# MariusFurter/WeightedSampling.jl

Measured on NVIDIA B200. Metric: particle_updates_per_sec, higher is better.
Workload: dtype f64

## Files before the change

include/wsb200.h:

```cpp
#ifndef WSB200_H
#define WSB200_H

#include <stdint.h>

#ifdef __cplusplus
extern "C" {
#endif

#define WSB200_ABI_VERSION 2

#define WS_OK 0
#define WS_EINVAL (-1)
#define WS_ENODEVICE (-2)
#define WS_ECUDA (-3)
#define WS_ENOMEM (-4)
#define WS_EUNSUPPORTED (-5)
#define WS_EREPLAY (-6)
#define WS_ENUMERIC (-7)
#define WS_ENCCL (-8)

typedef struct ws_ctx ws_ctx;

#define WS_RESAMPLER_STRATIFIED 0
#define WS_RESAMPLER_SYSTEMATIC 1
// ... 194 lines not shown
    int64_t h2d_bytes;
    int64_t d2h_bytes;
    double last_resample_ms;
    double last_pass_ms;
    int64_t sl_passes;
} ws_stats;
int ws_get_stats(ws_ctx* ctx, ws_stats* out);
int ws_get_clamped(ws_ctx* ctx, int64_t* out);
int ws_get_ess_ties(ws_ctx* ctx, int64_t* out);
#define WS_N_KERNEL_CLASSES 8
int ws_kernel_times(ws_ctx* ctx, double* ms_out, int64_t* count_out, int32_t n_classes);
int ws_reset_kernel_times(ws_ctx* ctx);
int ws_set_lazy_gather(ws_ctx* ctx, int on);
typedef struct ws_plane_stats {
    double mean, median, std, min, max;
    double hist[8];
} ws_plane_stats;
int ws_describe(ws_ctx* ctx, int32_t n_planes, const int32_t* col, const int32_t* comp, ws_plane_stats* out, double* ess);

int ws_set_genealogy(ws_ctx* ctx, int on, int64_t budget_bytes);
int ws_genealogy_info(ws_ctx* ctx, int64_t* n_vectors, int64_t* bytes, int64_t* events);
int ws_col_events_behind(ws_ctx* ctx, int32_t id, int64_t* out);
int ws_set_timing(ws_ctx* ctx, int on);
int ws_get_migrated(ws_ctx* ctx, int64_t* out);
int ws_get_pushed(ws_ctx* ctx, int64_t* out);
int ws_get_mailbox_exchanges(ws_ctx* ctx, int64_t* out);
int ws_get_traced_pushes(ws_ctx* ctx, int64_t* out);
int ws_next_philox_stream(ws_ctx* ctx, uint64_t* stream_out, uint64_t* seed_out);
int ws_stream(ws_ctx* ctx, void** stream_out);

#ifdef __cplusplus
}
#endif
#endif
```

weightedsampling.jl_b200/_lib.py:

```python
from __future__ import annotations

import ctypes as C
import os

_HERE = os.path.dirname(os.path.abspath(__file__))
LIB_PATH = os.environ.get("WSB200_LIB", os.path.join(_HERE, "lib", "libwsb200.so"))


class WsError(RuntimeError):

    def __init__(self, code, msg):
        super().__init__(f"wsb200 error {code}: {msg}")
        self.code = code
        self.msg = msg


class UnsupportedModelError(WsError):
    """The statement is outside the fixed device-op set (rejected, never run on the CPU)."""


WS_OK, WS_EINVAL, WS_ENODEVICE, WS_ECUDA, WS_ENOMEM, WS_EUNSUPPORTED, WS_EREPLAY, WS_ENUMERIC, WS_ENCCL = (
    0, -1, -2, -3, -4, -5, -6, -7, -8)

RESAMPLER = {"stratified": 0, "systematic": 1, "multinomial": 2}
# ... 121 lines not shown
    "ws_marginal_diversity": (C.c_int, [_ctx, C.c_int32, _i32p, _i32p, _dp]),
    "ws_score_logpdf": (C.c_int, [_ctx, C.c_int64, C.c_void_p]),
    "ws_tape_clear": (C.c_int, [_ctx]),
    "ws_tape_record_only": (C.c_int, [_ctx, C.c_int]),
    "ws_tape_length": (C.c_int, [_ctx, _i64p]),
    "ws_tape_enable": (C.c_int, [_ctx, C.c_int]),
    "ws_set_replay_normals": (C.c_int, [_ctx, C.c_void_p, C.c_int64]),
    "ws_set_replay_uniforms": (C.c_int, [_ctx, C.c_void_p, C.c_int64]),
    "ws_set_replay_exponentials": (C.c_int, [_ctx, C.c_void_p, C.c_int64]),
    "ws_set_replay_variates": (C.c_int, [_ctx, C.c_void_p, C.c_int64]),
    "ws_get_stats": (C.c_int, [_ctx, C.POINTER(ws_stats)]),
    "ws_get_clamped": (C.c_int, [_ctx, _i64p]),
    "ws_get_ess_ties": (C.c_int, [_ctx, _i64p]),
    "ws_kernel_times": (C.c_int, [_ctx, _dp, _i64p, C.c_int32]),
    "ws_reset_kernel_times": (C.c_int, [_ctx]),
    "ws_set_timing": (C.c_int, [_ctx, C.c_int]),
    "ws_set_lazy_gather": (C.c_int, [_ctx, C.c_int]),
    "ws_describe": (C.c_int, [_ctx, C.c_int32, C.POINTER(C.c_int32), C.POINTER(C.c_int32), C.POINTER(ws_plane_stats),
                              C.POINTER(C.c_double)]),
    "ws_set_genealogy": (C.c_int, [_ctx, C.c_int, C.c_int64]),
    "ws_genealogy_info": (C.c_int, [_ctx, _i64p, _i64p, _i64p]),
    "ws_col_events_behind": (C.c_int, [_ctx, C.c_int32, _i64p]),
    "ws_next_philox_stream": (C.c_int, [_ctx, C.POINTER(C.c_uint64), C.POINTER(C.c_uint64)]),
    "ws_get_migrated": (C.c_int, [_ctx, _i64p]),
    "ws_get_pushed": (C.c_int, [_ctx, _i64p]),
    "ws_get_mailbox_exchanges": (C.c_int, [_ctx, _i64p]),
    "ws_get_traced_pushes": (C.c_int, [_ctx, _i64p]),
    "ws_stream": (C.c_int, [_ctx, C.POINTER(C.c_void_p)]),
}

_lib = None


def load():
    global _lib
    if _lib is not None:
        return _lib
    if not os.path.exists(LIB_PATH):
        raise ImportError(
            f"{LIB_PATH} is missing: build it with `python -c 'import __graft_entry__ as g; g.build()'` "
            "(nvcc, sm_100a).  wsb200 has no CPU fallback.")
    if "WSB200_NCCL_LIB" not in os.environ:
        import importlib.util
        spec = importlib.util.find_spec("nvidia")
        for base in (list(spec.submodule_search_locations) if spec and spec.submodule_search_locations else []):
            cand = os.path.join(base, "nccl", "lib", "libnccl.so.2")
# ... 23 lines not shown
```

weightedsampling.jl_b200/csrc/ws_kernels.cu:

```cuda
#include "ws_internal.h"

static int g_sm_count = 148;

__device__ __forceinline__ void lse_push(WsLse& a, double l) {
    if (l == -INFINITY) return;
    if (l > a.m) {
        double sc = ws_exp_nonpos(a.m - l);
        a.S = a.S * sc + 1.0;
        a.Q = a.Q * sc * sc + 1.0;
        a.m = l;
    } else {
        double e = ws_exp_nonpos(l - a.m);
        a.S += e;
        a.Q += e * e;
    }
}

template <int K>
__device__ __forceinline__ void lse_push_many(WsLse& a, const double (&l)[K], const bool (&live)[K]) {
    double mx = -INFINITY;
#pragma unroll
    for (int j = 0; j < K; ++j)
        if (live[j]) mx = fmax(mx, l[j]);
    if (mx > a.m) {
// ... 556 lines not shown
int ws_vm_max_grid(int n_regs, int n_loads, int n_ops, int sm_count, int n_ckpt) {
    const int smem = ws_vm_smem_bytes(n_regs, n_loads, n_ops, n_ckpt) + 1024;
    int per_sm = (227 * 1024) / smem;
    if (per_sm > WS_VM_MINB) per_sm = WS_VM_MINB;
    if (per_sm < 1) per_sm = 1;
    return per_sm * sm_count;
}

cudaError_t ws_launch_vm(const WsVmProgram& P, int grid, cudaStream_t s) {
    if (!g_vm_interp_only && P.n_ckpt == 0) {
        switch (ws_sl_find(P)) {
#define WS_SL_CASE(idx, Sig) \
    case idx: return ws_launch_vm_sl<Sig>(P, s);
            WS_SL_SIGS(WS_SL_CASE)
#undef WS_SL_CASE
            default: break;
        }
    }
    if (!g_vm_interp_only && P.n_ckpt != 0 && ws_slck_ok(P)) {
        constexpr int smem_ck = WsSigLinregObs::n_loads * WS_VM_BLOCK * WS_SLCK_P * (int)sizeof(double);
        ws_vm_sl_ckpt_kernel<WsSigLinregObs, WS_SLCK_P, WS_SLCK_N><<<ws_slck_grid(P), WS_VM_BLOCK, smem_ck, s>>>(P);
        return cudaGetLastError();
    }
    const int smem = ws_vm_smem_bytes(P.n_regs, P.n_loads, P.n_ops, P.n_ckpt);
    if (P.n_ckpt > 0) {
        if (ws_vm_staged(P.n_regs, P.n_loads)) ws_vm_kernel<true, true><<<grid, WS_VM_BLOCK, smem, s>>>(P);
        else ws_vm_kernel<false, true><<<grid, WS_VM_BLOCK, smem, s>>>(P);
    } else if (ws_vm_staged(P.n_regs, P.n_loads)) ws_vm_kernel<true><<<grid, WS_VM_BLOCK, smem, s>>>(P);
    else ws_vm_kernel<false><<<grid, WS_VM_BLOCK, smem, s>>>(P);
    return cudaGetLastError();
}

__global__ void __launch_bounds__(256) ws_reduce_logw_kernel(const double* __restrict__ logw, int64_t n,
                                                             WsLse* __restrict__ partials) {
    __shared__ WsLse warp_scratch[8];
    WsLse part;
    part.m = -INFINITY;
    part.S = 0.0;
    part.Q = 0.0;
    const int64_t stride = (int64_t)gridDim.x * 256;
    for (int64_t i = (int64_t)blockIdx.x * 256 + threadIdx.x; i < n; i += stride) lse_push(part, __ldg(logw + i));
    WsLse tot = lse_block_reduce<256>(part, warp_scratch);
    if (threadIdx.x == 0) partials[blockIdx.x] = tot;
}

cudaError_t ws_launch_reduce_logw(const double* logw, int64_t n, WsLse* partials, int grid, cudaStream_t s) {
    ws_reduce_logw_kernel<<<grid, 256, 0, s>>>(logw, n, partials);
    return cudaGetLastError();
}

__device__ __forceinline__ void ws_count_ess_tie(double ess, double ess_min, unsigned long long* ties) {
    if (ties != nullptr && fabs(ess - ess_min) <= 8.0 * 2.220446049250313e-16 * fabs(ess_min)) atomicAdd(ties, 1ull);
// ... 1967 lines not shown
```

weightedsampling.jl_b200/csrc/ws_lowering.h:

```cpp
#pragma once
#include <math.h>
#include <stdint.h>
#include <string.h>
#include <map>
#include <string>
#include <utility>
#include <vector>
#include "../../include/wsb200.h"
#include "ws_vm.cuh"

namespace wsl {

struct Plane {
    int32_t col, comp;
    bool operator<(const Plane& o) const { return col < o.col || (col == o.col && comp < o.comp); }
    bool operator==(const Plane& o) const { return col == o.col && comp == o.comp; }
};

struct Val {
    bool is_const;
    double c0, c1;
    int reg;
    static Val constant(double v) { return Val{true, v, 0.0, -1}; }
    static Val lin(double c0, double c1, int reg) { return Val{false, c0, c1, reg}; }
// ... 799 lines not shown
    const double K = (-0.5 * WS_LOG2PI - log(ts)) - (-0.5 * WS_LOG2PI - log(ps));
    p.has_acc = true;
    p.emit(ws_make_op(WS_OP_ACC_LIN2, 0, st.reg, sp.reg, WS_REG_NONE, 0, K, -0.5, 0.5));
}

inline void stmt_sample_expr(Program& p, RngCursor& rc, Plane dst, const ws_expr& sampler, const ws_expr* weighter) {
    p.rng = &rc;
    Val x = p.compile(sampler);
    p.rng = nullptr;
    p.store_val(dst, x);
    if (weighter != nullptr) p.acc_val(p.compile(*weighter));
}

inline bool mvnormal_factors(int d, const double* cov, std::vector<double>& L, std::vector<double>& Linv, double& c0) {
    if (!cholesky_lower(d, cov, L)) return false;
    lower_inverse(d, L, Linv);
    double logdet = 0.0;
    for (int j = 0; j < d; ++j) logdet += log(L[j * d + j]);
    logdet *= 2.0;
    c0 = -((double)d * WS_LOG2PI + logdet) / 2.0;
    return true;
}

}
```

weightedsampling.jl_b200/csrc/ws_runtime.cu:

```cuda
#include <math.h>
#include <stdarg.h>
#include <stdio.h>
#include <string.h>
#include <algorithm>
#include <functional>
#include <memory>
#include <deque>
#include <map>
#include <string>
#include <vector>

#include <dlfcn.h>
#include <unistd.h>
#include <chrono>

#include "../../include/wsb200.h"
#include "ws_internal.h"
#include "ws_lowering.h"
#include "ws_move.h"
#include "ws_stats.h"
#include "ws_exchange.h"

using wsl::Plane;
using wsl::Program;
// ... 44 lines not shown
    WS_SYM(GetUniqueId, "ncclGetUniqueId")
    WS_SYM(CommInitRank, "ncclCommInitRank")
    WS_SYM(CommDestroy, "ncclCommDestroy")
    WS_SYM(AllGather, "ncclAllGather")
    WS_SYM(AllReduce, "ncclAllReduce")
    WS_SYM(Send, "ncclSend")
    WS_SYM(Recv, "ncclRecv")
    WS_SYM(GroupStart, "ncclGroupStart")
    WS_SYM(GroupEnd, "ncclGroupEnd")
    WS_SYM(GetErrorString, "ncclGetErrorString")
#undef WS_SYM
    g_nccl.handle = h;
    return true;
}

enum WsKernelClass { KC_VM = 0, KC_REDUCE, KC_FINALIZE, KC_SCAN, KC_GATHER, KC_FILL, KC_MOVE, KC_OTHER, KC_COUNT };

struct Column {
    std::string name;
    int32_t width;
    std::vector<double*> front, back;
    std::vector<uint8_t> stale;
    std::vector<int64_t> ep;
};

struct TimedEvent {
    int kclass;
    cudaEvent_t a, b;
};

struct TapeEntry {
    int64_t depth;
    int32_t op_end;
    int32_t cache_ops;
    double konst_end;
    std::function<void(Program&)> lower;
    std::vector<Plane> refs;
};

struct OwnedExprs {
    std::vector<std::vector<ws_tok>> toks;
    std::vector<ws_expr> ex;
    explicit OwnedExprs(std::initializer_list<std::pair<const ws_expr*, int>> groups) {
        for (auto& g : groups)
            for (int i = 0; i < g.second; ++i) toks.emplace_back(g.first[i].toks, g.first[i].toks + g.first[i].n);
        for (auto& t : toks) ex.push_back(ws_expr{t.data(), (int32_t)t.size(), 0});
// ... 86 lines not shown
    int32_t* d_map = nullptr;
    int64_t map_ep = -1, map_E = -1;
    bool lazy_gather = true;
    unsigned long long* d_tile_words = nullptr;
    unsigned long long* d_cdf_local = nullptr;
    unsigned int* d_tile_counter = nullptr;
    int32_t* d_heavy_F = nullptr;
    unsigned long long* d_mn = nullptr;
    int64_t mn_cap_slots = 0;
    int64_t heavy_cap_n = 0;
    int64_t n_tiles = 0;
    unsigned long long* d_counters = nullptr;

    Program win;
    Program score;
    std::vector<TapeEntry> tape;
    WsOp* d_score_ops = nullptr;
    size_t d_score_cap = 0, d_score_uploaded = 0;
    WsOp* d_seg_ops = nullptr;
    size_t d_seg_cap = 0;
    bool record_only = false;
    bool tape_enabled = true;
    bool score_wide = false;

    double* d_replay_n = nullptr;
    double* d_replay_u = nullptr;
    double* d_replay_e = nullptr;
    double* d_replay_v = nullptr;
    int64_t replay_v_len = 0, cur_v = 0;
    int64_t replay_n_len = 0, replay_u_len = 0, replay_e_len = 0;
    int64_t cur_n = 0, cur_u = 0, cur_e = 0;

    double* d_scratch = nullptr;
    void* d_scratch2 = nullptr;
    size_t scratch2_bytes = 0;
    size_t scratch_bytes = 0;
    double* h_scratch = nullptr;
    size_t h_scratch_bytes = 0;

    ncclComm_t comm = nullptr;
    double* d_all_msq = nullptr;
    unsigned long long* d_all_tot = nullptr;
    int32_t* d_all_bounds = nullptr;
    int32_t* d_anc_src = nullptr;
    int64_t anc_src_cap = 0;
    double* d_send = nullptr;
// ... 420 lines not shown
    if (c->h_scratch) cudaFreeHost(c->h_scratch);
    for (auto& te : c->pending_events) {
        cudaEventDestroy(te.a);
        cudaEventDestroy(te.b);
    }
    for (auto& ev : c->event_pool) {
        cudaEventDestroy(ev.first);
        cudaEventDestroy(ev.second);
    }
    if (c->stream) cudaStreamDestroy(c->stream);
    delete c;
    return WS_OK;
}

static double* plane_ptr(ws_ctx* c, Plane p) { return c->cols[p.col].front[p.comp]; }

static int check_plane(ws_ctx* c, int32_t col, int32_t comp) {
    if (col < 0 || col >= (int32_t)c->cols.size()) return fail(c, WS_EINVAL, "unknown column id %d", col);
    if (comp < 0 || comp >= c->cols[col].width)
        return fail(c, WS_EINVAL, "component %d out of range for column %s (width %d)", comp, c->cols[col].name.c_str(),
                    c->cols[col].width);
    return WS_OK;
}
static int check_expr(ws_ctx* c, const ws_expr* e, const char* what) {
    if (e == nullptr || e->toks == nullptr || e->n <= 0) return fail(c, WS_EINVAL, "%s: empty expression", what);
    for (int i = 0; i < e->n; ++i)
        if (e->toks[i].op == WS_TOK_PLANE) TRY(check_plane(c, e->toks[i].col, e->toks[i].comp));
    return WS_OK;
}

static int flush_window(ws_ctx* c) {
    Program& w = c->win;
    if (w.ops.empty() && w.dirty.empty()) {
        reset_window(c);
        return WS_OK;
    }
    if (c->spec_block && !c->spec_flushing)
        return fail(c, WS_EUNSUPPORTED, "a speculative block was interrupted by a flush of the statement window");
    CK(c, cudaSetDevice(c->device));
    WsVmProgram P;
    memset(&P, 0, sizeof(P));
    P.n = c->n;
    P.particle_offset = c->offset;
    P.n_ops = (int)w.ops.size();
    P.n_loads = (int)w.loads.size();
    P.n_stores = (int)w.dirty.size();
    P.n_regs = std::max(1, w.high_water);
    {
        std::vector<Plane> loaded;
        for (auto& ld : w.loads) loaded.push_back(ld.first);
        TRY(materialize_deep(c, loaded));
    }
    P.ancestors = c->d_anc;
    P.load_gather = 0u;
    std::vector<Plane> swap_after;
    for (int k = 0; k < P.n_loads; ++k) {
        const Plane pl = w.loads[k].first;
        P.load_ptr[k] = plane_ptr(c, pl);
        P.load_reg[k] = (uint8_t)w.loads[k].second;
        if (c->cols[pl.col].stale[pl.comp]) P.load_gather |= (1u << k);
    }
    for (int k = 0; k < P.n_stores; ++k) {
        const Plane pl = w.dirty[k];
        Column& col = c->cols[pl.col];
        P.store_reg[k] = (uint8_t)w.plane_reg[pl];
        bool loaded = false;
        for (auto& ld : w.loads)
            if (ld.first == pl) loaded = true;
        if (col.stale[pl.comp] && loaded) {
            if (col.back[pl.comp] == nullptr) TRY(pool_alloc(c, (void**)&col.back[pl.comp], sizeof(double) * (size_t)(c->n + c->spare)));
            P.store_ptr[k] = col.back[pl.comp];
            swap_after.push_back(pl);
        } else {
            P.store_ptr[k] = col.front[pl.comp];
        }
    }
    if (w.has_acc) {
        P.logw = c->logw;
        if (c->logw_spec) {
            P.logw_mode = 3;
            P.red = c->d_red;
        } else if (c->logw_uniform) {
            P.logw_mode = 2;
            P.logw_base = c->logw_base;
        } else {
            P.logw_mode = 1;
        }
    } else {
// ... 3 lines not shown
        P.n_ckpt = (int32_t)c->spec_steps.size();
        for (int32_t j = 0; j < P.n_ckpt; ++j) P.ckpt_pc[j] = (uint8_t)c->spec_steps[j].ckpt_pc;
        P.ckpt_partials = c->d_ck_partials;
        P.logw_out = c->d_logw_bak;
    }
    const int64_t vm_tile = (int64_t)WS_VM_BLOCK * WS_VM_P;
    const int grid = (int)std::min<int64_t>(ws_vm_max_grid(P.n_regs, P.n_loads, P.n_ops, c->sm_count, P.n_ckpt), (c->n + vm_tile - 1) / vm_tile);
    P.partials = w.has_acc ? c->d_partials : nullptr;
    P.n_expect = 0;
    P.rng.seed = c->seed;
    P.rng.replay_n = c->d_replay_n;
    P.rng.replay_u = c->d_replay_u;
    P.rng.replay_e = c->d_replay_e;
    P.rng.replay_v = c->d_replay_v;
    memcpy(P.ops, w.ops.data(), sizeof(WsOp) * w.ops.size());

    const int sl_grid = ws_vm_sl_grid(P);
    TimedEvent te;
    timed_begin(c, KC_VM, te);
    CK(c, ws_launch_vm(P, std::max(1, grid), c->stream));
    timed_end(c, te);
    if (sl_grid > 0) c->stats.sl_passes++;
    for (auto& pl : swap_after) std::swap(c->cols[pl.col].front[pl.comp], c->cols[pl.col].back[pl.comp]);
    for (auto& pl : w.dirty) {
        c->cols[pl.col].stale[pl.comp] = 0;
        c->cols[pl.col].ep[pl.comp] = c->epoch;
    }
    c->stats.fused_passes++;
    c->stats.fused_statements += w.n_statements;
    if (w.has_acc) {
        c->logw_uniform = false;
        c->logw_spec = false;
        c->partials_valid = true;
        c->n_partials = sl_grid > 0 ? sl_grid : std::max(1, grid);
        c->red_valid = false;
    }
    reset_window(c);
    return WS_OK;
}

extern "C" int ws_flush(ws_ctx* c) {
    if (!c) return WS_EINVAL;
    return flush_window(c);
}
extern "C" int ws_sync(ws_ctx* c) {
    if (!c) return WS_EINVAL;
    TRY(flush_window(c));
    CK(c, cudaStreamSynchronize(c->stream));
    TRY(resolve_spec(c));
// ... 125 lines not shown
    TRY(flush_window(c));
    c->depth = 0;
    c->spec_immediate = 0;
    reset_score(c);
    return WS_OK;
}

extern "C" int ws_col_ensure(ws_ctx* c, const char* name, int32_t width, int32_t* id_out) {
    if (!c || !name) return WS_EINVAL;
    if (width < 1 || width > 4096) return fail(c, WS_EINVAL, "column %s: width %d out of range", name, width);
    auto it = c->col_index.find(name);
    if (it != c->col_index.end()) {
        if (c->cols[it->second].width != width)
            return fail(c, WS_EINVAL, "column %s already exists with width %d (requested %d)", name, c->cols[it->second].width, width);
        if (id_out) *id_out = it->second;
        return WS_OK;
    }
    CK(c, cudaSetDevice(c->device));
    Column col;
    col.name = name;
    col.width = width;
    col.stale.assign((size_t)width, 0);
    col.ep.assign((size_t)width, c->epoch);
    for (int k = 0; k < width; ++k) {
        double *f = nullptr, *b = nullptr;
        TRY(pool_alloc(c, (void**)&f, sizeof(double) * (size_t)(c->n + c->spare)));
        if (c->nranks > 1) TRY(pool_alloc(c, (void**)&b, sizeof(double) * (size_t)(c->n + c->spare)));
        CK(c, cudaMemsetAsync(f, 0, sizeof(double) * (size_t)c->n, c->stream));
        col.front.push_back(f);
        col.back.push_back(b);
    }
    c->cols.push_back(col);
    const int32_t id = (int32_t)c->cols.size() - 1;
    c->col_index[name] = id;
    if (id_out) *id_out = id;
    return WS_OK;
}
extern "C" int ws_col_lookup(const ws_ctx* c, const char* name, int32_t* id_out, int32_t* width_out) {
    if (!c || !name) return WS_EINVAL;
    auto it = c->col_index.find(name);
    if (it == c->col_index.end()) {
        if (id_out) *id_out = -1;
        if (width_out) *width_out = 0;
        return WS_OK;
    }
    if (id_out) *id_out = it->second;
// ... 2 lines not shown
}
extern "C" int ws_col_count(const ws_ctx* c, int32_t* out) {
    if (!c || !out) return WS_EINVAL;
    *out = (int32_t)c->cols.size();
    return WS_OK;
}
extern "C" int ws_col_info(const ws_ctx* c, int32_t id, char* name_buf, int32_t name_buf_len, int32_t* width_out) {
    if (!c) return WS_EINVAL;
    if (id < 0 || id >= (int32_t)c->cols.size()) return WS_EINVAL;
    if (name_buf && name_buf_len > 0) {
        strncpy(name_buf, c->cols[id].name.c_str(), (size_t)name_buf_len - 1);
        name_buf[name_buf_len - 1] = 0;
    }
    if (width_out) *width_out = c->cols[id].width;
    return WS_OK;
}
extern "C" int ws_col_download(ws_ctx* c, int32_t id, double* host_out) {
    if (!c || !host_out) return WS_EINVAL;
    if (id < 0 || id >= (int32_t)c->cols.size()) return fail(c, WS_EINVAL, "unknown column id %d", id);
    TRY(flush_window(c));
    CK(c, cudaSetDevice(c->device));
    const Column& col = c->cols[id];
    for (int k = 0; k < col.width; ++k) {
        const double* src = col.front[k];
        const int32_t* map = nullptr;
        if (col.stale[k]) TRY(map_for_epoch(c, col.ep[k], &map));
        if (map != nullptr) {
            TRY(ensure_scratch(c, sizeof(double) * (size_t)c->n));
            WsGatherParams G;
            memset(&G, 0, sizeof(G));
            G.n = c->n;
            G.ancestors = map;
            G.n_planes = 1;
            G.src[0] = col.front[k];
            G.dst[0] = c->d_scratch;
            TimedEvent te;
            timed_begin(c, KC_GATHER, te);
            CK(c, ws_launch_gather(G, grid_for(c, c->n, 256, 8), c->stream));
            timed_end(c, te);
            src = c->d_scratch;
        }
        CK(c, cudaMemcpyAsync(host_out + (size_t)k * c->n, src, sizeof(double) * (size_t)c->n, cudaMemcpyDeviceToHost, c->stream));
        if (map != nullptr) CK(c, cudaStreamSynchronize(c->stream));
    }
    CK(c, cudaStreamSynchronize(c->stream));
    c->stats.d2h_bytes += (int64_t)sizeof(double) * c->n * col.width;
    return WS_OK;
}
extern "C" int ws_col_upload(ws_ctx* c, int32_t id, const double* host_in) {
    if (!c || !host_in) return WS_EINVAL;
    if (id < 0 || id >= (int32_t)c->cols.size()) return fail(c, WS_EINVAL, "unknown column id %d", id);
    TRY(flush_window(c));
    Column& col = c->cols[id];
    for (auto& st : col.stale) st = 0;
    for (auto& e : col.ep) e = c->epoch;
    for (int k = 0; k < col.width; ++k)
        CK(c, cudaMemcpyAsync(col.front[k], host_in + (size_t)k * c->n, sizeof(double) * (size_t)c->n, cudaMemcpyHostToDevice, c->stream));
    CK(c, cudaStreamSynchronize(c->stream));
    c->stats.h2d_bytes += (int64_t)sizeof(double) * c->n * col.width;
    return WS_OK;
}

static int materialize_logw(ws_ctx* c) {
    TRY(resolve_spec(c));
    if (!c->logw_uniform) return WS_OK;
    TimedEvent te;
    timed_begin(c, KC_FILL, te);
    CK(c, ws_launch_fill(c->logw, c->logw_base, c->n, grid_for(c, c->n, 256, 8), c->stream));
    timed_end(c, te);
    c->logw_uniform = false;
    c->partials_valid = false;
    return WS_OK;
}

extern "C" int ws_weights_download(ws_ctx* c, double* host_out) {
    if (!c || !host_out) return WS_EINVAL;
    TRY(flush_window(c));
    TRY(materialize_logw(c));
// ... 432 lines not shown
        TRY(map_for_epoch(c, g.first, &map));
        if (map == nullptr) {
            for (auto& pl : g.second) {
                c->cols[pl.col].stale[pl.comp] = 0;
                c->cols[pl.col].ep[pl.comp] = c->epoch;
            }
            continue;
        }
        TRY(gather_planes(c, map, g.second));
    }
    if (!only) c->anc_pending = false;
    return WS_OK;
}

static int materialize_tape_planes(ws_ctx* c, int32_t n_extra, const int32_t* col, const int32_t* comp) {
    std::vector<Plane> need;
    for (auto& ld : c->score.loads) need.push_back(ld.first);
    for (auto& te : c->tape)
        for (auto& pl : te.refs) need.push_back(pl);
    for (int32_t t = 0; t < n_extra; ++t) need.push_back(Plane{col[t], comp[t]});
    std::vector<Plane> ok;
    for (auto& pl : need)
        if (pl.col >= 0 && pl.col < (int32_t)c->cols.size() && pl.comp >= 0 && pl.comp < c->cols[pl.col].width) ok.push_back(pl);
    return materialize_planes(c, &ok);
}

static int materialize_deep(ws_ctx* c, const std::vector<Plane>& planes) {
    std::vector<Plane> deep;
    for (auto& pl : planes) {
        const Column& col = c->cols[pl.col];
        if (col.stale[pl.comp] && col.ep[pl.comp] < c->epoch - 1) deep.push_back(pl);
    }
    if (deep.empty()) return WS_OK;
    return materialize_planes(c, &deep);
}

static bool shard_genealogy_ok(const ws_ctx* c) { return c->push_exchange && c->push_min == 0; }
static int64_t spare_ring_cap(const ws_ctx* c, int q) {
    return ws_spare_rows(ws_rank_lo(c->n_global, c->nranks, q + 1) - ws_rank_lo(c->n_global, c->nranks, q));
}
static int prepare_resample_event(ws_ctx* c) {
    c->event_keeps = c->genealogy && c->lazy_gather && (c->nranks == 1 || shard_genealogy_ok(c));
    if (!c->event_keeps) {
        TRY(materialize_planes(c));
        for (auto& rg : c->spare_rings) rg.clear();
        return WS_OK;
// ... 52 lines not shown
    }
    if (c->anc_live.empty() && c->anc_pool.empty() && c->d_anc != nullptr) c->anc_pool.push_back(c->d_anc);
    int32_t* fresh = nullptr;
    if (!c->anc_pool.empty()) {
        fresh = c->anc_pool.back();
        c->anc_pool.pop_back();
    } else {
        const int64_t margin = c->nranks > 1 ? c->spare : 0;
        TRY(pool_alloc(c, (void**)&fresh, sizeof(int32_t) * (size_t)(c->n + c->spare + margin)));
        fresh += margin;
    }
    c->anc_live.push_back({c->epoch + 1, fresh});
    c->d_anc = fresh;
    return WS_OK;
}
static int begin_resample_event(ws_ctx* c) {
    TRY(prepare_resample_event(c));
    return commit_resample_event(c);
}

static void end_resample_event(ws_ctx* c) {
    c->epoch++;
    for (auto& col : c->cols)
        for (auto& st : col.stale) st = 1;
    c->anc_pending = !c->cols.empty();
}

static int gather_all(ws_ctx* c, const int32_t* d_anc) {
    std::vector<Plane> which;
    for (int32_t ci = 0; ci < (int32_t)c->cols.size(); ++ci)
        for (int32_t k = 0; k < c->cols[ci].width; ++k) which.push_back(Plane{ci, k});
    return gather_planes(c, d_anc, which);
}

static bool small_resample_ok(const ws_ctx* c, const double* d_ru) {
    return c->small_resample && c->nranks == 1 && c->n <= WS_SMALL_N && d_ru == nullptr && c->resampler != WS_RESAMPLER_MULTINOMIAL;
}
static int run_small_resample(ws_ctx* c, uint64_t stream_id, int gate, int do_finalize) {
    WsScanParams S;
    memset(&S, 0, sizeof(S));
    S.logw = c->logw;
    S.mode = 0;
    S.scheme = c->resampler;
    S.red = c->d_red;
    S.gate = gate;
    S.n = c->n;
    S.n_slots = c->n;
// ... 816 lines not shown
        TRY(begin_resample_event(c));
        TRY(run_scan_search(c, c->logw, 0, c->resampler, c->n, nullptr, nullptr, c->d_anc, c->d_tile_words, c->d_cdf_local, stream_id,
                            c->d_counters + 0, 1));
        end_resample_event(c);
    }
    c->spec_head++;
    c->spec_pending++;
    c->stats.resamples_fired++;
    c->logw_uniform = false;
    c->logw_spec = true;
    c->partials_valid = false;
    c->red_valid = false;
    c->weights_changed = false;
    c->last_info_pending = true;
    return WS_OK;
}

extern "C" int ws_exec(ws_ctx* c, const ws_cmd* cmds, int32_t n_cmds, const double* params, int32_t n_params) {
    if (!c || (!cmds && n_cmds > 0) || n_cmds < 0) return WS_EINVAL;
    std::vector<ws_tok> toks;
    std::vector<ws_expr> ex;
    for (int32_t k = 0; k < n_cmds; ++k) {
        const ws_cmd& cm = cmds[k];
        toks.clear();
        ex.clear();
        size_t first[3] = {0, 0, 0};
        std::vector<size_t> off;
        for (int a = 0; a < 3; ++a) {
            first[a] = ex.size();
            if (cm.n_e[a] < 0 || (cm.n_e[a] > 0 && cm.e[a] == nullptr)) return fail(c, WS_EINVAL, "ws_exec: command %d has a bad expression list", k);
            for (int32_t j = 0; j < cm.n_e[a]; ++j) {
                const ws_expr& src = cm.e[a][j];
                if (src.toks == nullptr || src.n <= 0) return fail(c, WS_EINVAL, "ws_exec: command %d has an empty expression", k);
                off.push_back(toks.size());
                for (int32_t i = 0; i < src.n; ++i) {
                    ws_tok t = src.toks[i];
                    if (t.op == WS_TOK_PARAM) {
                        if (t.col < 0 || t.col >= n_params || params == nullptr)
                            return fail(c, WS_EINVAL, "ws_exec: parameter %d of %d", t.col, n_params);
                        t.op = WS_TOK_CONST;
                        t.val = params[t.col];
                        t.col = 0;
                    }
                    toks.push_back(t);
                }
                ex.push_back(ws_expr{nullptr, src.n, 0});
// ... 3 lines not shown
        const ws_expr* e0 = cm.n_e[0] > 0 ? &ex[first[0]] : nullptr;
        const ws_expr* e1 = cm.n_e[1] > 0 ? &ex[first[1]] : nullptr;
        const ws_expr* e2 = cm.n_e[2] > 0 ? &ex[first[2]] : nullptr;
        switch (cm.fn) {
            case WS_CMD_ASSIGN: TRY(ws_assign(c, cm.i0, cm.i1, e0)); break;
            case WS_CMD_ASSIGN_VEC: TRY(ws_assign_vec(c, cm.i0, cm.i1, e0)); break;
            case WS_CMD_SAMPLE_NORMAL: TRY(ws_sample_normal(c, cm.i0, cm.i1, e0, e1)); break;
            case WS_CMD_SAMPLE_EXPONENTIAL: TRY(ws_sample_exponential(c, cm.i0, cm.i1, e0)); break;
            case WS_CMD_SAMPLE_MVNORMAL: TRY(ws_sample_mvnormal(c, cm.i0, cm.i1, e0, cm.mat)); break;
            case WS_CMD_OBSERVE_NORMAL: TRY(ws_observe_normal(c, e0, e1, e2)); break;
            case WS_CMD_OBSERVE_EXPONENTIAL: TRY(ws_observe_exponential(c, e0, e1)); break;
            case WS_CMD_OBSERVE_MVNORMAL: TRY(ws_observe_mvnormal(c, cm.i0, e0, e1, cm.mat)); break;
            case WS_CMD_WEIGHT_EXPR: TRY(ws_weight_expr(c, e0)); break;
            case WS_CMD_SAMPLE_EXPR: TRY(ws_sample_expr(c, cm.i0, cm.i1, e0, e1, e2)); break;
            case WS_CMD_RESAMPLE: TRY(ws_resample_async(c)); break;
            default: return fail(c, WS_EINVAL, "ws_exec: unknown command %d", cm.fn);
        }
    }
    return WS_OK;
}

extern "C" int ws_exec_n(ws_ctx* c, const ws_cmd* cmds, int32_t n_cmds, const double* params, int32_t n_params, int32_t n_elems) {
    if (!c || n_elems < 0 || (n_params > 0 && n_elems > 0 && !params)) return WS_EINVAL;
    for (int32_t e = 0; e < n_elems; ++e) TRY(ws_exec(c, cmds, n_cmds, params + (size_t)e * (size_t)n_params, n_params));
    return WS_OK;
}

static int spec_checkpoint(ws_ctx* c) {
    if (!c->weights_changed) return WS_OK;
    if (c->win.ops.empty() || !c->win.has_acc) return fail(c, WS_EUNSUPPORTED, "speculative block: a step without a weighting term");
    if (!c->win.dirty.empty()) return fail(c, WS_EUNSUPPORTED, "speculative block: a statement writes a column");
    if (c->spec_steps.size() >= WS_VM_MAX_CKPT) return fail(c, WS_EUNSUPPORTED, "speculative block: more than %d steps", WS_VM_MAX_CKPT);
    if (c->win.ops.size() > 255) return fail(c, WS_EUNSUPPORTED, "speculative block: window too long");
    ws_ctx::SpecStep st;
    st.tape_size = c->tape.size();
    st.score_mark = c->score.mark();
    st.depth = c->depth;
    st.stream_before = c->next_stream;
    st.ckpt_pc = (int32_t)c->win.ops.size() - 1;
    c->spec_steps.push_back(st);
    c->next_stream++;
    c->weights_changed = false;
    return WS_OK;
}

extern "C" int ws_exec_spec(ws_ctx* c, const ws_cmd* cmds, int32_t n_cmds, const double* params, int32_t n_params, int32_t n_steps,
                            int32_t* n_done, int32_t* fired) {
    if (!c || !n_done || !fired || n_steps < 1 || (n_params > 0 && !params)) return WS_EINVAL;
// ... 326 lines not shown
        else
            p.emit(ws_make_op(WS_OP_LIN2, t, v.reg, WS_REG_NONE, WS_REG_NONE, 0, v.c0, v.c1, 0));
        regs[k] = t;
        p.end_statement();
    }
    if (!p.error.empty()) return fail(c, WS_EINVAL, "%s", p.error.c_str());
    if (p.overflow) return fail(c, WS_EUNSUPPORTED, "ws_expectation: expressions do not fit one device pass");
    WsVmProgram P;
    memset(&P, 0, sizeof(P));
    P.n = c->n;
    P.particle_offset = c->offset;
    P.n_ops = (int)p.ops.size();
    P.n_loads = (int)p.loads.size();
    P.n_stores = 0;
    P.n_regs = std::max(1, p.high_water);
    {
        std::vector<Plane> loaded;
        for (auto& ld : p.loads) loaded.push_back(ld.first);
        TRY(materialize_deep(c, loaded));
    }
    P.ancestors = c->d_anc;
    for (int k = 0; k < P.n_loads; ++k) {
        const Plane pl = p.loads[k].first;
        P.load_ptr[k] = plane_ptr(c, pl);
        P.load_reg[k] = (uint8_t)p.loads[k].second;
        if (c->cols[pl.col].stale[pl.comp]) P.load_gather |= (1u << k);
    }
    P.logw_mode = 0;
    P.logw = c->logw;
    P.n_expect = n_exprs;
    for (int k = 0; k < n_exprs; ++k) P.expect_reg[k] = (uint8_t)regs[k];
    P.red = c->d_red;
    const int64_t vm_tile = (int64_t)WS_VM_BLOCK * WS_VM_P;
    const int grid = (int)std::max<int64_t>(1, std::min<int64_t>(ws_vm_max_grid(P.n_regs, P.n_loads, P.n_ops, c->sm_count), (c->n + vm_tile - 1) / vm_tile));
    TRY(ensure_scratch(c, sizeof(double) * (size_t)grid * 8));
    TRY(ensure_h_scratch(c, sizeof(double) * (size_t)grid * 8));
    P.expect_partials = c->d_scratch;
    P.rng.seed = c->seed;
    memcpy(P.ops, p.ops.data(), sizeof(WsOp) * p.ops.size());
    TimedEvent te;
    timed_begin(c, KC_VM, te);
    CK(c, ws_launch_vm(P, grid, c->stream));
    timed_end(c, te);
    CK(c, cudaMemcpyAsync(c->h_scratch, c->d_scratch, sizeof(double) * (size_t)grid * n_exprs, cudaMemcpyDeviceToHost, c->stream));
    CK(c, cudaStreamSynchronize(c->stream));
    for (int k = 0; k < n_exprs; ++k) {
        double s = 0.0;
        for (int b = 0; b < grid; ++b) s += c->h_scratch[(size_t)b * n_exprs + k];
        out[k] = s;
    }
    if (c->nranks > 1) TRY(allreduce_host_doubles(c, out, n_exprs));
    return WS_OK;
}

extern "C" int ws_col_download_rows(ws_ctx* c, int32_t id, const int64_t* indices, int64_t n_idx, double* host_out) {
    if (!c || !indices || !host_out || n_idx <= 0) return c ? fail(c, WS_EINVAL, "ws_col_download_rows: bad arguments") : WS_EINVAL;
    if (id < 0 || id >= (int32_t)c->cols.size()) return fail(c, WS_EINVAL, "unknown column id %d", id);
    for (int64_t i = 0; i < n_idx; ++i)
        if (indices[i] < 0 || indices[i] >= c->n) return fail(c, WS_EINVAL, "row index %lld out of range", (long long)indices[i]);
    TRY(flush_window(c));
    CK(c, cudaSetDevice(c->device));
    TempBuf idx, out, rows;
    CK(c, cudaMalloc(&idx.p, sizeof(int64_t) * (size_t)n_idx));
    CK(c, cudaMalloc(&out.p, sizeof(double) * (size_t)n_idx));
    CK(c, cudaMemcpyAsync(idx.p, indices, sizeof(int64_t) * (size_t)n_idx, cudaMemcpyHostToDevice, c->stream));
    const Column& col = c->cols[id];
    for (int k = 0; k < col.width; ++k) {
        const int64_t* use = (const int64_t*)idx.p;
        if (col.stale[k]) {
            if (rows.p == nullptr) CK(c, cudaMalloc(&rows.p, sizeof(int64_t) * (size_t)n_idx));
            const int64_t* start = (const int64_t*)idx.p;
            int64_t from = c->epoch;
            while (from > col.ep[k]) {
                WsComposeParams P;
                memset(&P, 0, sizeof(P));
                P.n = n_idx;
                P.n_rows = c->n;
                while (from > col.ep[k] && P.n_chain < WS_COMPOSE_MAX_CHAIN) {
                    const int32_t* a = anc_of_event(c, from);
                    if (a == nullptr) return fail(c, WS_EINVAL, "genealogy: ancestors of event %lld were released", (long long)from);
                    P.chain[P.n_chain++] = a;
                    --from;
                }
                CK(c, ws_launch_compose_rows(P, (int64_t*)rows.p, start, c->stream));
                c->stats.kernel_launches++;
                start = (const int64_t*)rows.p;
            }
            use = (const int64_t*)rows.p;
        }
        CK(c, ws_launch_gather_rows(col.front[k], use, n_idx, (double*)out.p, c->stream));
// ... 658 lines not shown
}

extern "C" int ws_describe(ws_ctx* c, int32_t n_planes, const int32_t* col, const int32_t* comp, ws_plane_stats* out, double* ess) {
    if (!c || !col || !comp || !out || n_planes < 1) return c ? fail(c, WS_EINVAL, "ws_describe: bad arguments") : WS_EINVAL;
    for (int t = 0; t < n_planes; ++t) TRY(check_plane(c, col[t], comp[t]));
    TRY(ensure_reduced(c));
    WsStatsComm comm{c, c->nranks, stats_allgather_words, stats_allreduce_doubles, stats_allreduce_u64_device};
    if (c->nranks > 1) {
        std::vector<Plane> pl;
        for (int t = 0; t < n_planes; ++t) pl.push_back(Plane{col[t], comp[t]});
        TRY(materialize_planes(c, &pl));
    }
    CK(c, cudaSetDevice(c->device));
    static_assert(sizeof(ws_plane_stats) == sizeof(WsPlaneStats), "ws_plane_stats layout");
    const size_t sb = ws_stats_scratch_bytes(c->n);
    const size_t q_off = (sb + 255) & ~(size_t)255;
    TRY(ensure_scratch(c, q_off + 16 * (size_t)c->n));
    TRY(ensure_h_scratch(c, sb));
    unsigned long long* d_q = (unsigned long long*)((char*)c->d_scratch + q_off);
    double* d_x = (double*)(d_q + c->n);
    CK(c, ws_stats_weights(c->logw, c->d_red, c->logw_uniform ? 1 : 0, c->n, c->n_global, d_q, c->stream));
    c->stats.kernel_launches++;
    for (int t = 0; t < n_planes; ++t) {
        const Column& cl = c->cols[col[t]];
        const double* x = cl.front[comp[t]];
        const int32_t* map = nullptr;
        if (cl.stale[comp[t]]) TRY(map_for_epoch(c, cl.ep[comp[t]], &map));
        if (map != nullptr) {
            WsGatherParams G;
            memset(&G, 0, sizeof(G));
            G.n = c->n;
            G.ancestors = map;
            G.n_planes = 1;
            G.src[0] = x;
            G.dst[0] = d_x;
            TimedEvent te;
            timed_begin(c, KC_GATHER, te);
            CK(c, ws_launch_gather(G, grid_for(c, c->n, 256, 8), c->stream));
            timed_end(c, te);
            x = d_x;
        }
        int launches = 0;
        WsPlaneStats ps;
        CK(c, ws_stats_plane(x, d_q, c->n, c->d_scratch, c->h_scratch, c->stream, &ps, &launches, c->nranks > 1 ? &comm : nullptr));
        c->stats.kernel_launches += launches;
        memcpy(&out[t], &ps, sizeof(ps));
// ... 27 lines not shown
    return WS_OK;
}
extern "C" int ws_next_philox_stream(ws_ctx* c, uint64_t* stream_out, uint64_t* seed_out) {
    if (!c) return WS_EINVAL;
    if (stream_out) *stream_out = c->next_stream;
    if (seed_out) *seed_out = c->seed;
    return WS_OK;
}
extern "C" int ws_get_traced_pushes(ws_ctx* c, int64_t* out) {
    if (!c || !out) return WS_EINVAL;
    *out = c->traced_rows;
    return WS_OK;
}
extern "C" int ws_get_mailbox_exchanges(ws_ctx* c, int64_t* out) {
    if (!c || !out) return WS_EINVAL;
    *out = c->mbox_on ? c->mbox_exchanges : 0;
    return WS_OK;
}
extern "C" int ws_get_pushed(ws_ctx* c, int64_t* out) {
    if (!c || !out) return WS_EINVAL;
    *out = c->pushed_total;
    return WS_OK;
}
extern "C" int ws_get_migrated(ws_ctx* c, int64_t* out) {
    if (!c || !out) return WS_EINVAL;
    *out = c->migrated_total;
    return WS_OK;
}
extern "C" int ws_stream(ws_ctx* c, void** stream_out) {
    if (!c || !stream_out) return WS_EINVAL;
    *stream_out = (void*)c->stream;
    return WS_OK;
}
```

weightedsampling.jl_b200/csrc/ws_vm_sl.cuh:

```cuda
#pragma once
#include <cmath>
#include <utility>
#include "ws_vm.cuh"
#if defined(__CUDACC__)
#include "ws_internal.h"
#endif

#if defined(__CUDACC__)
#define WS_SL_CX __host__ __device__ constexpr
#else
#define WS_SL_CX constexpr
#endif
struct WsSlOp {
    uint8_t op, dst, a, b, c;
    uint32_t imm;
    uint8_t kflags;
};
#define WS_SL_K0Z 1u
#define WS_SL_K1ONE 2u
#define WS_SL_K2ONE 4u
#define WS_SL_ADD (WS_SL_K0Z | WS_SL_K1ONE | WS_SL_K2ONE)

WS_SL_CX bool ws_sl_dst_is_reg(uint32_t op) {
    return !(op == WS_OP_LOGPDF_NORMAL || op == WS_OP_LOGPDF_EXPON || op == WS_OP_ACC_LIN2 || op == WS_OP_ACC_QUAD2 ||
// ... 204 lines not shown
    constexpr bool rnd = ws_sl_imm_is_runtime(s.op);
    d.k0 = (s.kflags & WS_SL_K0Z) ? 0.0 : kk[0];
    d.k1 = (s.kflags & WS_SL_K1ONE) ? 1.0 : (swap ? kk[2] : kk[1]);
    d.k2 = (s.kflags & WS_SL_K2ONE) ? 1.0 : kk[2];
    if (rnd && replay) {
        d.k1 = o.k1;
        d.k2 = o.k2;
    }
    ws_vm_exec_d<1, PP>(d, R, acc, rng, particle);
}
template <class Sig, int PP, int BLOCK, int K>
__device__ __forceinline__ void ws_sl_load1(double* __restrict__ R, const double* __restrict__ stage) {
    constexpr int r = Sig::load_reg[K];
#pragma unroll
    for (int j = 0; j < PP; ++j) R[r * PP + j] = stage[(K * PP + j) * BLOCK];
}
template <class Sig, int PP, int BLOCK, int... K>
__device__ __forceinline__ void ws_sl_loads(double* __restrict__ R, const double* __restrict__ stage, std::integer_sequence<int, K...>) {
    (ws_sl_load1<Sig, PP, BLOCK, K>(R, stage), ...);
}
template <class Sig, int PP, int BLOCK, int K>
__device__ __forceinline__ void ws_sl_store1(const double* __restrict__ R, const WsVmProgram& P, const unsigned first, const bool (&live)[PP]) {
    constexpr int r = Sig::store_reg[K];
    double* __restrict__ ptr = P.store_ptr[K] + first;
#pragma unroll
    for (int j = 0; j < PP; ++j)
        if (live[j]) ptr[j * BLOCK] = R[r * PP + j];
}
template <class Sig, int PP, int BLOCK, int... K>
__device__ __forceinline__ void ws_sl_stores(const double* __restrict__ R, const WsVmProgram& P, const unsigned first, const bool (&live)[PP],
                                             std::integer_sequence<int, K...>) {
    (ws_sl_store1<Sig, PP, BLOCK, K>(R, P, first, live), ...);
}
template <class Sig, int PP, int... I>
__device__ __forceinline__ void ws_sl_run(double* __restrict__ R, double (&acc)[PP], const WsVmProgram& P, const WsSlConsts<Sig>& K,
                                          const bool replay, const uint64_t (&particle)[PP], std::integer_sequence<int, I...>) {
    (ws_sl_step<Sig, I, PP>(R, acc, P.ops[I], K.k[I], replay, P.rng, particle), ...);
}
template <class Sig, int PP, int... I>
__device__ __forceinline__ void ws_sl_run_at(double* __restrict__ R, double (&acc)[PP], const WsVmProgram& P, const WsOp* ops,
                                             const WsSlConsts<Sig>& K, const uint64_t (&particle)[PP], std::integer_sequence<int, I...>) {
    (ws_sl_step<Sig, I, PP>(R, acc, ops[I], K.k[I], false, P.rng, particle), ...);
}
#endif
```

Baseline: 44.97 billion.

## Elide stores of planes overwritten before read across loop iterations

Adds a liveness analysis over the loop body in ws_exec_n that finds planes each command writes which are overwritten before any read in the following commands (wrapping around to the next iteration). Fused passes then skip global stores to those dead planes by nulling store pointers; the interpreter path compacts the store list and the specialized path checks for null. Dead planes are tracked per column so later reads of them raise an error and resampling does not gather them. This cuts memory write traffic at the cost of host-side analysis and extra bookkeeping.

```diff
diff --git a/include/wsb200.h b/include/wsb200.h
--- a/include/wsb200.h
+++ b/include/wsb200.h
@@ -240,6 +240,7 @@
 int ws_genealogy_info(ws_ctx* ctx, int64_t* n_vectors, int64_t* bytes, int64_t* events);
 int ws_col_events_behind(ws_ctx* ctx, int32_t id, int64_t* out);
 int ws_set_timing(ws_ctx* ctx, int on);
+int ws_get_elided_stores(ws_ctx* ctx, int64_t* out);
 int ws_get_migrated(ws_ctx* ctx, int64_t* out);
 int ws_get_pushed(ws_ctx* ctx, int64_t* out);
 int ws_get_mailbox_exchanges(ws_ctx* ctx, int64_t* out);
diff --git a/weightedsampling.jl_b200/_lib.py b/weightedsampling.jl_b200/_lib.py
--- a/weightedsampling.jl_b200/_lib.py
+++ b/weightedsampling.jl_b200/_lib.py
@@ -167,6 +167,7 @@
     "ws_genealogy_info": (C.c_int, [_ctx, _i64p, _i64p, _i64p]),
     "ws_col_events_behind": (C.c_int, [_ctx, C.c_int32, _i64p]),
     "ws_next_philox_stream": (C.c_int, [_ctx, C.POINTER(C.c_uint64), C.POINTER(C.c_uint64)]),
+    "ws_get_elided_stores": (C.c_int, [_ctx, _i64p]),
     "ws_get_migrated": (C.c_int, [_ctx, _i64p]),
     "ws_get_pushed": (C.c_int, [_ctx, _i64p]),
     "ws_get_mailbox_exchanges": (C.c_int, [_ctx, _i64p]),
diff --git a/weightedsampling.jl_b200/csrc/ws_kernels.cu b/weightedsampling.jl_b200/csrc/ws_kernels.cu
--- a/weightedsampling.jl_b200/csrc/ws_kernels.cu
+++ b/weightedsampling.jl_b200/csrc/ws_kernels.cu
@@ -602,12 +602,19 @@
         ws_vm_sl_ckpt_kernel<WsSigLinregObs, WS_SLCK_P, WS_SLCK_N><<<ws_slck_grid(P), WS_VM_BLOCK, smem_ck, s>>>(P);
         return cudaGetLastError();
     }
-    const int smem = ws_vm_smem_bytes(P.n_regs, P.n_loads, P.n_ops, P.n_ckpt);
-    if (P.n_ckpt > 0) {
-        if (ws_vm_staged(P.n_regs, P.n_loads)) ws_vm_kernel<true, true><<<grid, WS_VM_BLOCK, smem, s>>>(P);
-        else ws_vm_kernel<false, true><<<grid, WS_VM_BLOCK, smem, s>>>(P);
-    } else if (ws_vm_staged(P.n_regs, P.n_loads)) ws_vm_kernel<true><<<grid, WS_VM_BLOCK, smem, s>>>(P);
-    else ws_vm_kernel<false><<<grid, WS_VM_BLOCK, smem, s>>>(P);
+    WsVmProgram Q = P;
+    Q.n_stores = 0;
+    for (int k = 0; k < P.n_stores; ++k)
+        if (P.store_ptr[k] != nullptr) {
+            Q.store_ptr[Q.n_stores] = P.store_ptr[k];
+            Q.store_reg[Q.n_stores++] = P.store_reg[k];
+        }
+    const int smem = ws_vm_smem_bytes(Q.n_regs, Q.n_loads, Q.n_ops, Q.n_ckpt);
+    if (Q.n_ckpt > 0) {
+        if (ws_vm_staged(Q.n_regs, Q.n_loads)) ws_vm_kernel<true, true><<<grid, WS_VM_BLOCK, smem, s>>>(Q);
+        else ws_vm_kernel<false, true><<<grid, WS_VM_BLOCK, smem, s>>>(Q);
+    } else if (ws_vm_staged(Q.n_regs, Q.n_loads)) ws_vm_kernel<true><<<grid, WS_VM_BLOCK, smem, s>>>(Q);
+    else ws_vm_kernel<false><<<grid, WS_VM_BLOCK, smem, s>>>(Q);
     return cudaGetLastError();
 }
 
diff --git a/weightedsampling.jl_b200/csrc/ws_lowering.h b/weightedsampling.jl_b200/csrc/ws_lowering.h
--- a/weightedsampling.jl_b200/csrc/ws_lowering.h
+++ b/weightedsampling.jl_b200/csrc/ws_lowering.h
@@ -845,4 +845,57 @@
     return true;
 }
 
-}
+inline std::vector<std::vector<Plane>> body_dead_planes(const ws_cmd* cmds, int32_t n) {
+    struct Access {
+        std::vector<Plane> reads, writes;
+        bool known = true;
+    };
+    std::vector<Access> acc((size_t)n);
+    for (int32_t j = 0; j < n; ++j) {
+        const ws_cmd& cm = cmds[j];
+        Access& a = acc[(size_t)j];
+        for (int x = 0; x < 3 && a.known; ++x) {
+            if (cm.n_e[x] < 0 || (cm.n_e[x] > 0 && cm.e[x] == nullptr)) a.known = false;
+            for (int32_t i = 0; a.known && i < cm.n_e[x]; ++i) {
+                const ws_expr& ex = cm.e[x][i];
+                if (ex.toks == nullptr || ex.n <= 0) a.known = false;
+                for (int32_t t = 0; a.known && t < ex.n; ++t)
+                    if (ex.toks[t].op == WS_TOK_PLANE) a.reads.push_back(Plane{ex.toks[t].col, ex.toks[t].comp});
+            }
+        }
+        switch (cm.fn) {
+            case WS_CMD_ASSIGN:
+            case WS_CMD_SAMPLE_NORMAL:
+            case WS_CMD_SAMPLE_EXPONENTIAL:
+            case WS_CMD_SAMPLE_EXPR: a.writes.push_back(Plane{cm.i0, cm.i1}); break;
+            case WS_CMD_ASSIGN_VEC:
+            case WS_CMD_SAMPLE_MVNORMAL:
+                if (cm.i1 < 1 || cm.i1 > 4096) a.known = false;
+                for (int32_t q = 0; a.known && q < cm.i1; ++q) a.writes.push_back(Plane{cm.i0, q});
+                break;
+            case WS_CMD_OBSERVE_NORMAL:
+            case WS_CMD_OBSERVE_EXPONENTIAL:
+            case WS_CMD_OBSERVE_MVNORMAL:
+            case WS_CMD_WEIGHT_EXPR:
+            case WS_CMD_RESAMPLE: break;
+            default: a.known = false;
+        }
+    }
+    std::vector<std::vector<Plane>> dead((size_t)n);
+    for (int32_t k = 0; k < n; ++k) {
+        std::map<Plane, bool> seen;
+        if (!acc[(size_t)k].known) continue;
+        for (auto& pl : acc[(size_t)k].reads) seen.emplace(pl, false);
+        for (int32_t s = k + 1; s < k + 1 + n; ++s) {
+            const Access& a = acc[(size_t)(s % n)];
+            if (!a.known) break;
+            for (auto& pl : a.reads) seen.emplace(pl, false);
+            for (auto& pl : a.writes) seen.emplace(pl, true);
+        }
+        for (auto& kv : seen)
+            if (kv.second) dead[(size_t)k].push_back(kv.first);
+    }
+    return dead;
+}
+
+}
diff --git a/weightedsampling.jl_b200/csrc/ws_runtime.cu b/weightedsampling.jl_b200/csrc/ws_runtime.cu
--- a/weightedsampling.jl_b200/csrc/ws_runtime.cu
+++ b/weightedsampling.jl_b200/csrc/ws_runtime.cu
@@ -90,6 +90,7 @@
     std::vector<double*> front, back;
     std::vector<uint8_t> stale;
     std::vector<int64_t> ep;
+    std::vector<uint8_t> dead;
 };
 
 struct TimedEvent {
@@ -222,6 +223,9 @@
     bool record_only = false;
     bool tape_enabled = true;
     bool score_wide = false;
+    const std::vector<std::vector<Plane>>* body_dead = nullptr;
+    int32_t body_cmd = 0;
+    int64_t elided_stores = 0;
 
     double* d_replay_n = nullptr;
     double* d_replay_u = nullptr;
@@ -688,6 +692,12 @@
                     c->cols[col].width);
     return WS_OK;
 }
+static int check_live(ws_ctx* c, Plane p) {
+    if (c->cols[p.col].dead[p.comp])
+        return fail(c, WS_EINVAL, "column %s, component %d has no value: a loop element failed before it was written again",
+                    c->cols[p.col].name.c_str(), p.comp);
+    return WS_OK;
+}
 static int check_expr(ws_ctx* c, const ws_expr* e, const char* what) {
     if (e == nullptr || e->toks == nullptr || e->n <= 0) return fail(c, WS_EINVAL, "%s: empty expression", what);
     for (int i = 0; i < e->n; ++i)
@@ -722,14 +732,22 @@
     std::vector<Plane> swap_after;
     for (int k = 0; k < P.n_loads; ++k) {
         const Plane pl = w.loads[k].first;
+        TRY(check_live(c, pl));
         P.load_ptr[k] = plane_ptr(c, pl);
         P.load_reg[k] = (uint8_t)w.loads[k].second;
         if (c->cols[pl.col].stale[pl.comp]) P.load_gather |= (1u << k);
     }
+    const std::vector<Plane>* dead = (c->body_dead != nullptr && c->nranks == 1) ? &(*c->body_dead)[(size_t)c->body_cmd] : nullptr;
+    std::vector<uint8_t> elided((size_t)P.n_stores, 0);
     for (int k = 0; k < P.n_stores; ++k) {
         const Plane pl = w.dirty[k];
         Column& col = c->cols[pl.col];
         P.store_reg[k] = (uint8_t)w.plane_reg[pl];
+        if (dead != nullptr && std::find(dead->begin(), dead->end(), pl) != dead->end()) {
+            P.store_ptr[k] = nullptr;
+            elided[(size_t)k] = 1;
+            continue;
+        }
         bool loaded = false;
         for (auto& ld : w.loads)
             if (ld.first == pl) loaded = true;
@@ -779,9 +797,12 @@
     timed_end(c, te);
     if (sl_grid > 0) c->stats.sl_passes++;
     for (auto& pl : swap_after) std::swap(c->cols[pl.col].front[pl.comp], c->cols[pl.col].back[pl.comp]);
-    for (auto& pl : w.dirty) {
+    for (size_t k = 0; k < w.dirty.size(); ++k) {
+        const Plane pl = w.dirty[k];
         c->cols[pl.col].stale[pl.comp] = 0;
         c->cols[pl.col].ep[pl.comp] = c->epoch;
+        c->cols[pl.col].dead[pl.comp] = elided[k];
+        c->elided_stores += elided[k];
     }
     c->stats.fused_passes++;
     c->stats.fused_statements += w.n_statements;
@@ -953,6 +974,7 @@
     col.width = width;
     col.stale.assign((size_t)width, 0);
     col.ep.assign((size_t)width, c->epoch);
+    col.dead.assign((size_t)width, 0);
     for (int k = 0; k < width; ++k) {
         double *f = nullptr, *b = nullptr;
         TRY(pool_alloc(c, (void**)&f, sizeof(double) * (size_t)(c->n + c->spare)));
@@ -1001,6 +1023,7 @@
     CK(c, cudaSetDevice(c->device));
     const Column& col = c->cols[id];
     for (int k = 0; k < col.width; ++k) {
+        TRY(check_live(c, Plane{id, k}));
         const double* src = col.front[k];
         const int32_t* map = nullptr;
         if (col.stale[k]) TRY(map_for_epoch(c, col.ep[k], &map));
@@ -1033,6 +1056,7 @@
     Column& col = c->cols[id];
     for (auto& st : col.stale) st = 0;
     for (auto& e : col.ep) e = c->epoch;
+    for (auto& d : col.dead) d = 0;
     for (int k = 0; k < col.width; ++k)
         CK(c, cudaMemcpyAsync(col.front[k], host_in + (size_t)k * c->n, sizeof(double) * (size_t)c->n, cudaMemcpyHostToDevice, c->stream));
     CK(c, cudaStreamSynchronize(c->stream));
@@ -1511,6 +1535,7 @@
     std::vector<Plane> ok;
     for (auto& pl : need)
         if (pl.col >= 0 && pl.col < (int32_t)c->cols.size() && pl.comp >= 0 && pl.comp < c->cols[pl.col].width) ok.push_back(pl);
+    for (auto& pl : ok) TRY(check_live(c, pl));
     return materialize_planes(c, &ok);
 }
 
@@ -1609,7 +1634,12 @@
 static void end_resample_event(ws_ctx* c) {
     c->epoch++;
     for (auto& col : c->cols)
-        for (auto& st : col.stale) st = 1;
+        for (int k = 0; k < col.width; ++k) {
+            if (col.dead[k])
+                col.ep[k] = c->epoch;
+            else
+                col.stale[k] = 1;
+        }
     c->anc_pending = !c->cols.empty();
 }
 
@@ -2472,6 +2502,7 @@
     std::vector<ws_expr> ex;
     for (int32_t k = 0; k < n_cmds; ++k) {
         const ws_cmd& cm = cmds[k];
+        c->body_cmd = k;
         toks.clear();
         ex.clear();
         size_t first[3] = {0, 0, 0};
@@ -2521,8 +2552,15 @@
 
 extern "C" int ws_exec_n(ws_ctx* c, const ws_cmd* cmds, int32_t n_cmds, const double* params, int32_t n_params, int32_t n_elems) {
     if (!c || n_elems < 0 || (n_params > 0 && n_elems > 0 && !params)) return WS_EINVAL;
-    for (int32_t e = 0; e < n_elems; ++e) TRY(ws_exec(c, cmds, n_cmds, params + (size_t)e * (size_t)n_params, n_params));
-    return WS_OK;
+    if (n_cmds < 0 || (!cmds && n_cmds > 0)) return WS_EINVAL;
+    const std::vector<std::vector<Plane>> dead = n_elems > 1 ? wsl::body_dead_planes(cmds, n_cmds) : std::vector<std::vector<Plane>>();
+    int rc = WS_OK;
+    for (int32_t e = 0; e < n_elems && rc == WS_OK; ++e) {
+        c->body_dead = e + 1 < n_elems ? &dead : nullptr;
+        rc = ws_exec(c, cmds, n_cmds, params + (size_t)e * (size_t)n_params, n_params);
+    }
+    c->body_dead = nullptr;
+    return rc;
 }
 
 static int spec_checkpoint(ws_ctx* c) {
@@ -2895,6 +2933,7 @@
     P.ancestors = c->d_anc;
     for (int k = 0; k < P.n_loads; ++k) {
         const Plane pl = p.loads[k].first;
+        TRY(check_live(c, pl));
         P.load_ptr[k] = plane_ptr(c, pl);
         P.load_reg[k] = (uint8_t)p.loads[k].second;
         if (c->cols[pl.col].stale[pl.comp]) P.load_gather |= (1u << k);
@@ -2939,6 +2978,7 @@
     CK(c, cudaMemcpyAsync(idx.p, indices, sizeof(int64_t) * (size_t)n_idx, cudaMemcpyHostToDevice, c->stream));
     const Column& col = c->cols[id];
     for (int k = 0; k < col.width; ++k) {
+        TRY(check_live(c, Plane{id, k}));
         const int64_t* use = (const int64_t*)idx.p;
         if (col.stale[k]) {
             if (rows.p == nullptr) CK(c, cudaMalloc(&rows.p, sizeof(int64_t) * (size_t)n_idx));
@@ -3643,6 +3683,7 @@
     CK(c, ws_stats_weights(c->logw, c->d_red, c->logw_uniform ? 1 : 0, c->n, c->n_global, d_q, c->stream));
     c->stats.kernel_launches++;
     for (int t = 0; t < n_planes; ++t) {
+        TRY(check_live(c, Plane{col[t], comp[t]}));
         const Column& cl = c->cols[col[t]];
         const double* x = cl.front[comp[t]];
         const int32_t* map = nullptr;
@@ -3716,6 +3757,11 @@
     *out = c->pushed_total;
     return WS_OK;
 }
+extern "C" int ws_get_elided_stores(ws_ctx* c, int64_t* out) {
+    if (!c || !out) return WS_EINVAL;
+    *out = c->elided_stores;
+    return WS_OK;
+}
 extern "C" int ws_get_migrated(ws_ctx* c, int64_t* out) {
     if (!c || !out) return WS_EINVAL;
     *out = c->migrated_total;
diff --git a/weightedsampling.jl_b200/csrc/ws_vm_sl.cuh b/weightedsampling.jl_b200/csrc/ws_vm_sl.cuh
--- a/weightedsampling.jl_b200/csrc/ws_vm_sl.cuh
+++ b/weightedsampling.jl_b200/csrc/ws_vm_sl.cuh
@@ -250,6 +250,7 @@
 template <class Sig, int PP, int BLOCK, int K>
 __device__ __forceinline__ void ws_sl_store1(const double* __restrict__ R, const WsVmProgram& P, const unsigned first, const bool (&live)[PP]) {
     constexpr int r = Sig::store_reg[K];
+    if (P.store_ptr[K] == nullptr) return;
     double* __restrict__ ptr = P.store_ptr[K] + first;
 #pragma unroll
     for (int j = 0; j < PP; ++j)
```

Measured after the change: 46.79 billion (median of 6 runs). +4.0%, better.
